# Fanchuana/OPUS-PLLM

Measured on AMD Instinct MI355X. Metric: proteins_per_sec, higher is better.
Workload: dtype f16; 1 GPU; OPUS-PLLM-llama3_8b shape: batch 64/GPU, 512-residue proteins, 89-id prompt (+8 protein tokens = 96 positions), 32 new tokens, greedy (BASELINE configs[3] per-GPU shard: batch 512 over 8 GPUs); batch_per_gpu=64, residues=512, parallelism=replicas x1 (batch-sharded), all-gather of ids

## Files before the change

opus-pllm_amd/csrc/api.cpp:

```cpp
#include "../../include/opus_pllm.h"
#include "common.h"

#include <cmath>
#include <cstdarg>
#include <cstdio>
#include <cstdlib>
#include <cstring>
#include <algorithm>
#include <atomic>
#include <map>
#include <string>
#include <vector>

using namespace opus;

static thread_local char g_err[512] = "";
static int fail(int code, const char *fmt, ...) {
    va_list ap;
    va_start(ap, fmt);
    vsnprintf(g_err, sizeof(g_err), fmt, ap);
    va_end(ap);
    return code;
}
#define HIPC(expr)                                                                                   \
// ... 2409 lines not shown
}

extern "C" int opus_debug_attn_decode(opus_ctx *c, const void *d_qkv, const void *d_k_hist, const void *d_v_hist,
                                      const int32_t *d_kstart, int32_t B, int32_t T0, int32_t step, void *d_out, void *d_k_new,
                                      void *d_v_new, void *stream) {
    if (!c || !d_qkv || !d_kstart || !d_out) return fail(OPUS_EBADARG, "debug_attn_decode: null pointer");
    const opus_config &g = c->cfg;
    const int L = T0 + step, nkv = g.dec_kv_heads, hd = g.dec_head_dim;
    if (B < 1 || B > g.max_batch || T0 < 1 || T0 > g.max_prompt || step < 0 || step >= g.max_new_tokens)
        return fail(OPUS_ESHAPE, "debug_attn_decode: B=%d T0=%d step=%d exceed the context (%d, %d, %d)", B, T0, step, g.max_batch,
                    g.max_prompt, g.max_new_tokens);
    if (L > 0 && (!d_k_hist || !d_v_hist)) return fail(OPUS_EBADARG, "debug_attn_decode: history is null");
    HIPC(hipSetDevice(c->device));
    hipStream_t s = (hipStream_t)stream;
    const size_t pitch = (size_t)c->cache_sh * sizeof(half_t), roww = (size_t)L * hd * sizeof(half_t);
    HIPC(hipMemcpy2DAsync(c->kc, pitch, d_k_hist, roww, roww, (size_t)B * nkv, hipMemcpyDeviceToDevice, s));
    HIPC(hipMemcpy2DAsync(c->vc, pitch, d_v_hist, roww, roww, (size_t)B * nkv, hipMemcpyDeviceToDevice, s));
    HIPC(hipMemcpyAsync(c->d_kstart, d_kstart, (size_t)B * sizeof(int32_t), hipMemcpyDeviceToDevice, s));
    OPC(reset_step(c, s, T0, step));
    HIPC(launch_embed_tokens(c->d_next, nullptr, B, 0, 1, c->d_xl, nullptr, nullptr, 0, c->cs_dec, c->d_kstart, c->d_step, -1, hd / 2,
                             c->cs_row, nullptr, 0, s));
    AttnDecodeParams a;
    a.qkv = (const half_t *)d_qkv; a.slabs = nullptr; a.ks = 0; a.slab_stride = 0; a.row_ssq = nullptr; a.row_nblk = 0; a.eps = 0.f; a.K = 0;
    a.bias = nullptr;
    a.cs_row = c->cs_row; a.kstart = c->d_kstart; a.step = c->d_step; a.T0 = -1; a.nh = g.dec_heads; a.nkv = nkv;
    a.kc = c->kc; a.vc = c->vc; a.cache_sb = c->cache_sb; a.cache_sh = c->cache_sh;
    a.ctx_cap = g.max_prompt + g.max_new_tokens; a.scale = 1.0f / sqrtf((float)hd); a.out = (half_t *)d_out; a.out_tiled = 0;
    c->phase = PH_DECODE;
    KL(KC_ATTN_DECODE, 4.0 * B * nkv * hd * (L + 1), launch_attn_decode(a, B, hd, s));
    const size_t one = (size_t)hd * sizeof(half_t);
    if (d_k_new) HIPC(hipMemcpy2DAsync(d_k_new, one, c->kc + (size_t)L * hd, pitch, one, (size_t)B * nkv, hipMemcpyDeviceToDevice, s));
    if (d_v_new) HIPC(hipMemcpy2DAsync(d_v_new, one, c->vc + (size_t)L * hd, pitch, one, (size_t)B * nkv, hipMemcpyDeviceToDevice, s));
    c->prefilled = false;
    new_epoch(c);
    return OPUS_OK;
}

extern "C" int opus_debug_knob(opus_ctx *c, const char *name, int32_t value) {
    if (!name) return fail(OPUS_EBADARG, "debug_knob: null name");
    if (c) drop_graphs(c);
    if (!strcmp(name, "no_stream")) g_knobs.no_stream = value;
    else if (!strcmp(name, "debug_a_tiled")) g_knobs.debug_a_tiled = value;
    else if (!strcmp(name, "no_ln_fusion")) g_knobs.no_ln_fusion = value;
    else if (!strcmp(name, "enc_full_last_layer")) g_knobs.enc_full_last_layer = value;
    else if (!strcmp(name, "poison_handoff")) {
        if (!c) return fail(OPUS_EBADARG, "poison_handoff needs a context");
        std::vector<int32_t> h(HANDOFF_ERR, 0);
        if (value) for (int i = 0; i < HANDOFF_ERR; ++i) h[i] = i < 512 ? value : ((i & 1) ? 0 : 1);
        HIPC(hipSetDevice(c->device));
        HIPC(hipDeviceSynchronize());
        HIPC(hipMemcpy(c->d_cnt, h.data(), h.size() * sizeof(int32_t), hipMemcpyHostToDevice));
    }
    else if (!strcmp(name, "pp_gm")) { if (value < 1 || value > 64) return fail(OPUS_EBADARG, "pp_gm out of range"); g_knobs.pp_gm = value; }
    else if (!strncmp(name, "misc", 4) && name[4] >= '0' && name[4] <= '7' && !name[5]) g_knobs.misc[name[4] - '0'] = value;
    else return fail(OPUS_EBADARG, "debug_knob: unknown knob '%s'", name);
    return OPUS_OK;
}

extern "C" int64_t opus_stat(opus_ctx *c, const char *name) {
    if (!c || !name) return -1;
    if (!strcmp(name, "graph_instantiations")) return c->graph_instantiations;
    if (!strcmp(name, "graph_replays")) return c->graph_replays;
    if (!strcmp(name, "graphs_cached")) return (int64_t)c->graphs.size();
    if (!strcmp(name, "decode_steps")) return c->decode_steps;
    return -1;
}

extern "C" int opus_timing_enable(opus_ctx *c, int32_t on) {
    if (!c) return fail(OPUS_EBADARG, "ctx is null");
    c->timing = on != 0;
    return OPUS_OK;
}
extern "C" int opus_timing_reset(opus_ctx *c) {
    if (!c) return fail(OPUS_EBADARG, "ctx is null");
    HIPC(hipDeviceSynchronize());
    timing_clear(c);
    return OPUS_OK;
}
static const char *kclass_names[KC_COUNT] = {"gemm_skinny", "gemm_mid", "gemm_wide", "gemm_ring", "gemm_pp", "gemm_tile", "splitk_reduce",
                                            "attn_prefill", "attn_decode", "norm", "other", "gemm_stream", "contact", "constraint", "logitproc",
                                            "xent"};
static const char *phase_names[PH_COUNT] = {"encode", "project", "splice", "prefill", "decode", "other", "score"};

extern "C" int opus_timing_get(opus_ctx *c, const char *kernel_class, const char *phase, double *ms, int64_t *launches,
                               double *bytes, double *flops) {
    if (!c || !kernel_class || !phase || !ms || !launches || !bytes || !flops) return fail(OPUS_EBADARG, "null argument");
    int k = -1, ph = -1;
    const bool any_k = !strcmp(kernel_class, "*"), any_p = !strcmp(phase, "*");
    for (int i = 0; i < KC_COUNT; ++i) if (!strcmp(kclass_names[i], kernel_class)) k = i;
    for (int i = 0; i < PH_COUNT; ++i) if (!strcmp(phase_names[i], phase)) ph = i;
    if (k < 0 && !any_k) return fail(OPUS_EBADARG, "unknown kernel class '%s'", kernel_class);
    if (ph < 0 && !any_p) return fail(OPUS_EBADARG, "unknown phase '%s'", phase);
    HIPC(hipDeviceSynchronize());
    double t = 0, b = 0, f = 0;
    int64_t n = 0;
    for (auto &r : c->recs) {
        if ((!any_k && r.klass != k) || (!any_p && r.phase != ph)) continue;
        float e = 0;
        HIPC(hipEventElapsedTime(&e, r.e0, r.e1));
        t += e;
        b += r.bytes;
        f += r.flops;
        ++n;
    }
    *ms = t;
    *launches = n;
// ... 15 lines not shown
```

opus-pllm_amd/csrc/common.h:

```cpp
#pragma once
#include <hip/hip_runtime.h>
#include <hip/hip_ext.h>
#include <stdint.h>

namespace opus {

#ifdef OPUS_BF16
typedef __bf16 half_t;
typedef __bf16 h8 __attribute__((ext_vector_type(8)));
typedef __bf16 h4 __attribute__((ext_vector_type(4)));
typedef __bf16 h2 __attribute__((ext_vector_type(2)));
#else
typedef _Float16 half_t;
typedef _Float16 h8 __attribute__((ext_vector_type(8)));
typedef _Float16 h4 __attribute__((ext_vector_type(4)));
typedef _Float16 h2 __attribute__((ext_vector_type(2)));
#endif
typedef float f4 __attribute__((ext_vector_type(4)));
__device__ __forceinline__ f4 mfma16(h8 a, h8 b, f4 c) {
#ifdef OPUS_BF16
    return __builtin_amdgcn_mfma_f32_16x16x32_bf16(a, b, c, 0, 0, 0);
#else
    return __builtin_amdgcn_mfma_f32_16x16x32_f16(a, b, c, 0, 0, 0);
#endif
// ... 39 lines not shown
hipError_t ensure_dyn_lds(const void *fn, size_t bytes);

__device__ __forceinline__ void rotate_pair(float a, float b, float c, float sn, float &lo, float &hi) {
    lo = __builtin_fmaf(a, c, -__fmul_rn(b, sn));
    hi = __builtin_fmaf(b, c, __fmul_rn(a, sn));
    asm volatile("" : "+v"(lo), "+v"(hi));
}

__host__ __device__ __forceinline__ int64_t tiled_off(int row, int k, int K) {
    return ((int64_t)(row >> 4) * (K >> 6) + (k >> 6)) * 1024 + ((k & 63) >> 5) * 512 + ((((k & 31) >> 3) << 4) + (row & 15)) * 8 + (k & 7);
}

constexpr int HANDOFF_WORDS = 1024, HANDOFF_ERR = 1023;
constexpr int HANDOFF_SPIN_LIMIT = 1 << 19;

struct GemmParams {
    const half_t *A;
    const float *Af;
    float norm_eps;
    int64_t lda;
    const half_t *W;
    int M, N, K;
    const float *bias;
    const float *residual;
    int64_t ldr;
    void *C;
    int64_t ldc;
    int out_f32;
    int epi;
    float *ws;
    int64_t ws_bytes;
    half_t *xh_out;
    float *ssq_out;
    int *fused_done;
    const float *row_ssq;
    int row_nblk;
    int64_t ssq_cap = 0;
    int *nblk_out = nullptr;
    int slab_only = 0;
    int *ks_out = nullptr;
    int force_wide = 0;
    const float *rope_cs = nullptr;
    const int32_t *rope_pos = nullptr;
    int rope_T = 0, rope_cols = 0, rope_qcols = 0;
    float rope_qscale = 1.0f;
    int *rope_done = nullptr;
    int a_tiled = 0, xh_tiled = 0, c_tiled = 0;
    int *combine_cnt = nullptr;
    float *ln_part = nullptr;
    int *ln_done = nullptr;
    const float *ln_stat = nullptr;
    const float *ln_colsum = nullptr;
    int pp_gm = 8;
    int stagger = 0;
    int no_rot = 0;
    long long *trace = nullptr;
    int *pp_plan = nullptr;
};
constexpr int PP_PLAN_WORDS = 5;
enum PpTail { PP_TAIL_NONE = 0, PP_TAIL_PAIR = 1, PP_TAIL_REDUCE = 2 };

struct AttnParams {
    const half_t *Q, *K, *V;
    int64_t q_sb, q_st, k_sb, k_st, v_sb, v_st;
    half_t *O;
    int64_t o_sb, o_st;
    const int32_t *kstart;
    const int32_t *kend;
    int B, T, heads, group, head_dim, causal;
    float scale;
    const int32_t *cu = nullptr;
    int q_trim = 0;
};

hipError_t launch_gemm(const GemmParams &p, hipStream_t s, int *klass);
hipError_t launch_splitk_reduce(const GemmParams &p, int ks, hipStream_t s);
bool gemm_stream_ok(const GemmParams &p);
bool gemm_stream_would(int M, int N, int K, int slab_only, int a_tiled, int row_scale, int64_t ws_bytes);
hipError_t launch_gemm_stream(const GemmParams &p, hipStream_t s);
struct Knobs {
    int no_stream = 0;
    int no_ln_fusion = 0;
    int debug_a_tiled = 0;
    int pp_gm = 8;
    int enc_full_last_layer = 0;
    int misc[8] = {0, 0, 0, 0, 0, 0, 0, 0};
};
extern Knobs g_knobs;
template <int NWAVES, int ROWS>
__device__ __forceinline__ void block_row_rstd(const float *__restrict__ ssq, int M, int nblk, float inv_k, float eps, float *out,
                                               int wave, int lane) {
    constexpr int RW = (ROWS + NWAVES - 1) / NWAVES;
    float part[RW];
#pragma unroll
    for (int r = 0; r < RW; ++r) part[r] = 0.f;
    for (int j0 = 0; j0 < nblk; j0 += 256) {
        float t[RW][4];
#pragma unroll
        for (int r = 0; r < RW; ++r) {
            int row = wave + NWAVES * r;
            row = row < M ? row : M - 1;
#pragma unroll
            for (int u = 0; u < 4; ++u) {
                const int j = j0 + 64 * u + lane;
                t[r][u] = ssq[(int64_t)row * nblk + (j < nblk ? j : nblk - 1)];
                t[r][u] = j < nblk ? t[r][u] : 0.f;
            }
        }
#pragma unroll
        for (int r = 0; r < RW; ++r) part[r] += (t[r][0] + t[r][1]) + (t[r][2] + t[r][3]);
    }
#pragma unroll
    for (int r = 0; r < RW; ++r) {
        float q = part[r];
#pragma unroll
        for (int o = 32; o > 0; o >>= 1) q += __shfl_xor(q, o, 64);
        const int row = wave + NWAVES * r;
        if (lane == 0 && row < ROWS) out[row] = rsqrtf(q * inv_k + eps);
    }
}
bool gemm_goes_wide(int M, int N);
bool gemm_goes_pp(int M, int N);
hipError_t launch_attn_prefill(const AttnParams &p, hipStream_t s);
struct AttnPrefixParams {
    const half_t *kc, *vc;
    int64_t cache_sb, cache_sh;
    const int32_t *kstart;
    int Tp;
    const half_t *qkv;
    int n;
    const int32_t *list, *off, *blocks;
    half_t *out;
    int nh, nkv, hd;
    float scale;
    const int32_t *par = nullptr;
};
int attn_prefix_blocks(const int32_t *off, int P, int G, int n, int32_t *blocks);
// ... 170 lines not shown
```

opus-pllm_amd/csrc/gemm.hip:

```cpp
#include "common.h"
#include <cstdlib>
#include <map>
#include <type_traits>
#include <mutex>
#include <utility>

namespace opus {

thread_local LaunchEvents *tl_launch_ev = nullptr;
static Knobs knobs_from_env() {
    Knobs k;
    for (int i = 0; i < 8; ++i) {
        char name[32];
        snprintf(name, sizeof(name), "OPUS_KNOB_MISC%d", i);
        if (const char *v = getenv(name)) k.misc[i] = atoi(v);
    }
    return k;
}
Knobs g_knobs = knobs_from_env();

hipError_t ensure_dyn_lds(const void *fn, size_t bytes) {
    static std::mutex mu;
    static std::map<std::pair<int, const void *>, size_t> done;
    int dev = 0;
    hipError_t e = hipGetDevice(&dev);
    if (e != hipSuccess) return e;
    std::lock_guard<std::mutex> lock(mu);
    size_t &have = done[std::make_pair(dev, fn)];
    if (bytes <= have) return hipSuccess;
    e = hipFuncSetAttribute(fn, hipFuncAttributeMaxDynamicSharedMemorySize, (int)bytes);
    if (e == hipSuccess) have = bytes;
    return e;
}

__device__ __forceinline__ float gelu_erf(float x) {
    const float z = fabsf(x) * 0.70710678118654752f;
    const float t = __builtin_amdgcn_rcpf(1.0f + 0.3275911f * z);
    const float poly = t * (0.254829592f + t * (-0.284496736f + t * (1.421413741f + t * (-1.453152027f + t * 1.061405429f))));
    const float erf_abs = 1.0f - poly * __expf(-z * z);
    return 0.5f * x * (1.0f + copysignf(erf_abs, x));
}
__device__ __forceinline__ float silu(float x) { return x * __builtin_amdgcn_rcpf(1.0f + __expf(-x)); }

template <int MT, int EPI, bool NORM, bool ALDS>
__global__ __launch_bounds__(1024) void gemm_skinny_kernel(GemmParams p) {
    extern __shared__ __attribute__((aligned(16))) float red[];
    OPUS_ARGS_ONE_BATCH(p);
    constexpr int PB = EPI == EPI_SILU_GU16 ? 2 : 1;
    const int tid = threadIdx.x;
    const int lane = tid & 63;
    const int wave = __builtin_amdgcn_readfirstlane(tid >> 6);
    const int nwaves = blockDim.x >> 6;
    const int wpp = nwaves / PB;
    const int pl = PB == 1 ? 0 : wave / wpp, kpart = wave - pl * wpp;
    const int chunks = p.K >> 6;
    const int npanels = (p.N + 15) >> 4;
    int panel = blockIdx.x * PB + pl;
    panel = panel < npanels ? panel : npanels - 1;
    const int c0 = kpart_begin(chunks, kpart, wpp);
    const int c1 = kpart_begin(chunks, kpart + 1, wpp);
    const int g = lane >> 4, li = lane & 15;
    float *rss = red + nwaves * MT * 256;
    float *wss = rss + nwaves * MT * 16;
    half_t *xs = reinterpret_cast<half_t *>(wss + 256);
// ... 713 lines not shown
        if (ks + 1 < KS) read_frags(ks + 1, na, nb);
        __builtin_amdgcn_sched_barrier(0);
        mfmas(ca, cb, 1, TM);
        __builtin_amdgcn_s_setprio(0);
    };
    h8 a0[TM], b0[TN], a1[TM], b1[TN];
#pragma unroll
    for (int s = 0; s < NS; ++s)
        if (s < KS) stage_load(s);
    wait_glds(issued_upto(NS - 1));
    __builtin_amdgcn_s_barrier();
    read_frags(0, a0, b0);
    for (int ks = 0; ks < KS; ks += 2) {
        step(ks, a0, b0, a1, b1);
        if (ks + 1 < KS) step(ks + 1, a1, b1, a0, b0);
    }

    if (ksplit > 1) {
        float *slab = p.ws + (int64_t)ky * p.M * p.N;
#pragma unroll
        for (int i = 0; i < TM; ++i) {
            const int m = m0 + wm * (16 * TM) + i * 16 + li;
            if (m >= p.M) continue;
#pragma unroll
            for (int j = 0; j < TN; ++j) {
                const int nb = n0 + wn * (16 * TN) + j * 16 + 4 * g;
                if ((p.N & 3) == 0 && nb + 3 < p.N) {
                    *reinterpret_cast<float4 *>(slab + (int64_t)m * p.N + nb) = make_float4(acc[i][j][0], acc[i][j][1], acc[i][j][2], acc[i][j][3]);
                } else {
#pragma unroll
                    for (int r = 0; r < 4; ++r)
                        if (nb + r < p.N) slab[(int64_t)m * p.N + nb + r] = acc[i][j][r];
                }
            }
        }
        return;
    }
#pragma unroll
    for (int i = 0; i < TM; ++i) {
        const int m = m0 + wm * (16 * TM) + i * 16 + li;
        if (m >= p.M) continue;
        if (EPI == EPI_SILU_GU16) {
#pragma unroll
            for (int jj = 0; jj < TN / 2; ++jj)
                store4<EPI>(p, m, n0 + wn * (16 * TN) + jj * 32 + 4 * g, acc[i][2 * jj], acc[i][2 * jj + 1]);
        } else {
#pragma unroll
            for (int j = 0; j < TN; ++j) store4<EPI>(p, m, n0 + wn * (16 * TN) + j * 16 + 4 * g, acc[i][j], acc[i][j]);
        }
    }
}

constexpr int PP_DIST = 6;

__host__ __device__ __forceinline__ void pp_tile_coords(int id, int tiles_m, int tiles_n, int &tm, int &tn, int GM = 8) {
    const int per_group = GM * tiles_n;
    const int grp = id / per_group, rem_id = id - grp * per_group;
    const int rows_here = (tiles_m - grp * GM) < GM ? (tiles_m - grp * GM) : GM;
    tm = grp * GM + rem_id % rows_here;
    tn = rem_id / rows_here;
}
template <int EPI, bool LNA>
__device__ __forceinline__ void pp_finish(const GemmParams &p, f4 (&acc)[8][4], char *smem, const int wave, const int m0, const int n0,
                                          const int bid, const int full_tiles, const int tail_split, const int kpart, const bool partial);
template <int EPI, bool LNA>
__device__ __forceinline__ void pp_epilogue(const GemmParams &p, f4 (&acc)[8][4], char *smem, const int wave, const int m0, const int n0,
                                            const char *pair_slab);
template <int EPI, bool LNA = false>
__global__ __launch_bounds__(512) void gemm_pp_kernel(GemmParams p, int tiles_m, int tiles_n, int full_tiles, int tail_split) {
    extern __shared__ __attribute__((aligned(16))) char smem[];
    constexpr int HT = 16384;
    const int tid = threadIdx.x, lane = tid & 63;
    const int wave = __builtin_amdgcn_readfirstlane(tid >> 6);
    const int wr = wave >> 2, wc = wave & 3;
    const int g = lane >> 4, li = lane & 15;
    if (p.stagger > 0 && blockIdx.x < 256 && ((blockIdx.x >> 3) & 1))
        for (int i = 0; i < p.stagger; ++i) __builtin_amdgcn_s_sleep(127);
    if (p.trace && tid == 0) p.trace[blockIdx.x * 4] = wall_clock64();
    int bid = blockIdx.x, kpart = 0;
    const bool partial = bid >= full_tiles;
    if (!partial) {
        const int nwg = full_tiles, q = nwg >> 3, rr = nwg & 7, xcd = bid & 7;
        bid = (xcd < rr ? xcd * (q + 1) : rr * (q + 1) + (xcd - rr) * q) + (bid >> 3);
    } else {
        const int j = bid - full_tiles;
        bid = full_tiles + j / tail_split;
        kpart = j % tail_split;
    }
    int tm, tn;
    pp_tile_coords(bid, tiles_m, tiles_n, tm, tn, p.pp_gm);
    const int m0 = tm * 256, n0 = tn * 256;
    const int KT_all = p.K >> 6;
    const int kt0 = partial ? (int)((int64_t)KT_all * kpart / tail_split) : 0;
    const int kt1 = partial ? (int)((int64_t)KT_all * (kpart + 1) / tail_split) : KT_all;
    const int KT = kt1 - kt0, NH = 4 * KT;
    const int npanels = (p.N + 15) >> 4;

    typedef const __attribute__((address_space(1))) void *gptr_t;
    typedef __attribute__((address_space(3))) void *lptr_t;
    unsigned offA[2][2], offB[2][2];
#pragma unroll
    for (int j = 0; j < 2; ++j) {
        const int q = 2 * wave + j;
        const int lr = 8 * q + (lane >> 3);
        const int chunk = (lane & 7) ^ ((lr >> 1) & 7);
#pragma unroll
        for (int rh = 0; rh < 2; ++rh) {
            int row = m0 + (lr >> 6) * 128 + rh * 64 + (lr & 63);
            row = row < p.M ? row : p.M - 1;
            offA[j][rh] = (unsigned)(((int64_t)row * p.lda + chunk * 8) * 2);
        }
        const int pi = q >> 1, s = q & 1;
#pragma unroll
        for (int ch = 0; ch < 2; ++ch) {
            int pn = (n0 >> 4) + (pi >> 1) * 4 + ch * 2 + (pi & 1);
            pn = pn < npanels ? pn : npanels - 1;
            offB[j][ch] = (unsigned)((((int64_t)pn * KT_all) * 1024 + s * 512 + lane * 8) * 2);
        }
    }
    const char *baseA = reinterpret_cast<const char *>(p.A) + (int64_t)kt0 * 128;
    const char *baseB = reinterpret_cast<const char *>(p.W) + (int64_t)kt0 * 2048;
    auto issue_half = [&](int hq) {
        const int kt = hq >> 2, i = hq & 3;
        char *dst = smem + (hq & 7) * HT + (2 * wave) * 1024;
        const char *sa = baseA + (int64_t)kt * 128, *sb = baseB + (int64_t)kt * 2048;
#pragma unroll
        for (int j = 0; j < 2; ++j) {
            const char *src = (i == 0 || i == 3) ? sa + offA[j][i == 3] : sb + offB[j][i == 2];
            __builtin_amdgcn_global_load_lds((gptr_t)src, (lptr_t)(dst + j * 1024), 16, 0, 0);
        }
    };

// ... 10 lines not shown
#pragma unroll
        for (int s = 0; s < 2; ++s) aoff[rt][s] = lr * 128 + (((4 * s + g) ^ ((lr >> 1) & 7)) << 4);
    }
    const int boff = (wc * 2) * 2048 + lane * 16;
    auto read_a = [&](int kt, int rh, h8 (&af)[4][2]) {
        const char *base = smem + (4 * (kt & 1) + (rh ? 3 : 0)) * HT;
#pragma unroll
        for (int rt = 0; rt < 4; ++rt)
#pragma unroll
            for (int s = 0; s < 2; ++s) af[rt][s] = *reinterpret_cast<const h8 *>(base + aoff[rt][s]);
    };
    auto read_b = [&](int kt, int ch, h8 (&bf)[2][2]) {
        const char *base = smem + (4 * (kt & 1) + 1 + ch) * HT + boff;
#pragma unroll
        for (int ct = 0; ct < 2; ++ct)
#pragma unroll
            for (int s = 0; s < 2; ++s) bf[ct][s] = *reinterpret_cast<const h8 *>(base + ct * 2048 + s * 1024);
    };
    auto mfma_quadrant = [&](int rh, int ch, const h8 (&af)[4][2], const h8 (&bf)[2][2]) {
        asm volatile("s_waitcnt lgkmcnt(0)" ::: "memory");
        __builtin_amdgcn_s_setprio(1);
#pragma unroll
        for (int rt = 0; rt < 4; ++rt)
#pragma unroll
            for (int ct = 0; ct < 2; ++ct)
#pragma unroll
                for (int s = 0; s < 2; ++s) {
#pragma unroll
                    for (int rhh = 0; rhh < 2; ++rhh)
#pragma unroll
                        for (int chh = 0; chh < 2; ++chh)
                            if (rhh == rh && chh == ch)
                                acc[4 * rhh + rt][2 * chh + ct] =
                                    mfma16(bf[ct][s], af[rt][s], acc[4 * rhh + rt][2 * chh + ct]);
                }
        __builtin_amdgcn_s_setprio(0);
    };
    constexpr int D = PP_DIST;
    auto feed = [&](int phi) {
        if (phi + D < NH) {
            issue_half(phi + D);
            vmcnt_wait<2 * (D - 2)>();
        } else {
            const int left = NH - 1 - (phi + 2);
            if (left >= 3) vmcnt_wait<6>();
            else if (left == 2) vmcnt_wait<4>();
            else if (left == 1) vmcnt_wait<2>();
            else vmcnt_wait<0>();
        }
    };

#pragma unroll
    for (int h = 0; h < D; ++h)
        if (h < NH) issue_half(h);
    if (NH >= D) vmcnt_wait<2 * (D - 4)>();
    else vmcnt_wait<0>();
    __builtin_amdgcn_s_barrier();
    if (p.trace && tid == 0) p.trace[blockIdx.x * 4 + 1] = wall_clock64();
    if (wr == 1) __builtin_amdgcn_s_barrier();
    read_a(0, 0, a0);

    for (int kt = 0; kt < KT; ++kt) {
        const int phi = 4 * kt;
        read_b(kt, 0, b0);
        feed(phi);
        __builtin_amdgcn_s_barrier();
        mfma_quadrant(0, 0, a0, b0);
        __builtin_amdgcn_s_barrier();
        read_b(kt, 1, b1);
        feed(phi + 1);
        __builtin_amdgcn_s_barrier();
        mfma_quadrant(0, 1, a0, b1);
        __builtin_amdgcn_s_barrier();
        read_a(kt, 1, a1);
        feed(phi + 2);
        __builtin_amdgcn_s_barrier();
        mfma_quadrant(1, 1, a1, b1);
        __builtin_amdgcn_s_barrier();
        if (kt + 1 < KT) read_a(kt + 1, 0, a0);
        feed(phi + 3);
        __builtin_amdgcn_s_barrier();
        mfma_quadrant(1, 0, a1, b0);
        __builtin_amdgcn_s_barrier();
    }
    if (wr == 0) __builtin_amdgcn_s_barrier();
    if (p.trace && tid == 0) p.trace[blockIdx.x * 4 + 2] = wall_clock64();
    pp_finish<EPI, LNA>(p, acc, smem, wave, m0, n0, bid, full_tiles, tail_split, kpart, partial);
}

template <int EPI, bool LNA>
__device__ __forceinline__ void pp_finish(const GemmParams &p, f4 (&acc)[8][4], char *smem, const int wave, const int m0, const int n0,
                                          const int bid, const int full_tiles, const int tail_split, const int kpart, const bool partial) {
    int lane;
    asm volatile("v_mbcnt_lo_u32_b32 %0, -1, 0\n\tv_mbcnt_hi_u32_b32 %0, -1, %0" : "=v"(lane));
    const int tid = wave * 64 + lane;
    const int wr = wave >> 2, wc = wave & 3;
    const int g = lane >> 4, li = lane & 15;

    const char *pair_slab = nullptr;
    if (partial && tail_split == 2 && p.combine_cnt) {
        typedef unsigned int u4p __attribute__((ext_vector_type(4)));
        const int tt = bid - full_tiles;
        int *cnt = p.combine_cnt + 512 + 2 * tt;
        int *word = reinterpret_cast<int *>(smem);
        if (tid == 0) *word = __hip_atomic_fetch_add(cnt, 1, __ATOMIC_RELAXED, __HIP_MEMORY_SCOPE_AGENT);
        __syncthreads();
        const int order = *word;
        __syncthreads();
        if (order > 1 && tid == 0)
            __hip_atomic_store(p.combine_cnt + HANDOFF_ERR, 1, __ATOMIC_RELAXED, __HIP_MEMORY_SCOPE_AGENT);
        const __amdgpu_buffer_rsrc_t srs = __builtin_amdgcn_make_buffer_rsrc((void *)(p.ws + ((int64_t)tt << 16)), 0, 1 << 18, 0x00020000);
        if (order == 0) {
#pragma unroll
            for (int i = 0; i < 8; ++i)
#pragma unroll
                for (int j = 0; j < 4; ++j)
                    __builtin_amdgcn_raw_buffer_store_b128(__builtin_bit_cast(u4p, acc[i][j]), srs, ((i * 4 + j) * 512 + tid) * 16, 0, 16);
            asm volatile("s_waitcnt vmcnt(0)" ::: "memory");
            __syncthreads();
            if (tid == 0) __hip_atomic_store(cnt + 1, 1, __ATOMIC_RELAXED, __HIP_MEMORY_SCOPE_AGENT);
            return;
        }
        if (tid == 0) {
            int spins = 0;
            while (__hip_atomic_load(cnt + 1, __ATOMIC_RELAXED, __HIP_MEMORY_SCOPE_AGENT) == 0) {
                __builtin_amdgcn_s_sleep(4);
                if (++spins > HANDOFF_SPIN_LIMIT) {
                    __hip_atomic_store(p.combine_cnt + HANDOFF_ERR, 1, __ATOMIC_RELAXED, __HIP_MEMORY_SCOPE_AGENT);
                    break;
                }
            }
            __hip_atomic_store(cnt, 0, __ATOMIC_RELAXED, __HIP_MEMORY_SCOPE_AGENT);
            __hip_atomic_store(cnt + 1, 0, __ATOMIC_RELAXED, __HIP_MEMORY_SCOPE_AGENT);
        }
        __syncthreads();
        pair_slab = reinterpret_cast<const char *>(p.ws + ((int64_t)tt << 16));
    } else if (partial) {
        float *slab = p.ws + (((int64_t)(bid - full_tiles) * tail_split + kpart) << 16);
#pragma unroll
        for (int i = 0; i < 8; ++i) {
            const int r = wr * 128 + i * 16 + li;
#pragma unroll
            for (int j = 0; j < 4; ++j)
                *reinterpret_cast<float4 *>(slab + r * 256 + wc * 64 + j * 16 + 4 * g) = make_float4(acc[i][j][0], acc[i][j][1], acc[i][j][2], acc[i][j][3]);
        }
        return;
    }
    pp_epilogue<EPI, LNA>(p, acc, smem, wave, m0, n0, pair_slab);
}

template <int EPI, bool LNA>
__device__ __forceinline__ void pp_epilogue(const GemmParams &p, f4 (&acc)[8][4], char *smem, const int wave, const int m0, const int n0,
                                            const char *pair_slab) {
    int lane;
    asm volatile("v_mbcnt_lo_u32_b32 %0, -1, 0\n\tv_mbcnt_hi_u32_b32 %0, -1, %0" : "=v"(lane));
    const int tid = wave * 64 + lane;
    const int wr = wave >> 2, wc = wave & 3;
    const int g = lane >> 4, li = lane & 15;
    constexpr int NO = EPI == EPI_SILU_GU16 ? 32 : 64;
    const int nlim = EPI == EPI_SILU_GU16 ? p.N / 2 : p.N;
    const int nw0 = EPI == EPI_SILU_GU16 ? (n0 >> 1) + wc * 32 : n0 + wc * 64;
    const bool rows16 = ((p.ldc & 7) == 0) && ((p.ldr & 3) == 0) && nw0 + NO <= nlim;
    const __amdgpu_buffer_rsrc_t psrs = __builtin_amdgcn_make_buffer_rsrc((void *)pair_slab, 0, pair_slab ? 1 << 18 : 0, 0x00020000);
    auto pair_load = [&](int i, int j) {
        return __builtin_bit_cast(f4, __builtin_amdgcn_raw_buffer_load_b128(psrs, ((i * 4 + j) * 512 + tid) * 16, 0, 16));
    };
    if (!rows16) {
#pragma unroll
        for (int i = 0; i < 8; ++i) {
            f4 av[4];
#pragma unroll
            for (int j = 0; j < 4; ++j) av[j] = acc[i][j];
            if (pair_slab) {
#pragma unroll
                for (int j = 0; j < 4; ++j) av[j] += pair_load(i, j);
            }
            const int m = m0 + wr * 128 + i * 16 + li;
            if (m >= p.M) continue;
            if (EPI == EPI_SILU_GU16) {
#pragma unroll
                for (int jj = 0; jj < 2; ++jj) store4<EPI>(p, m, n0 + wc * 64 + jj * 32 + 4 * g, av[2 * jj], av[2 * jj + 1]);
            } else {
#pragma unroll
                for (int j = 0; j < 4; ++j) store4<EPI>(p, m, n0 + wc * 64 + j * 16 + 4 * g, av[j], av[j]);
            }
        }
        return;
    }
    float *patch = reinterpret_cast<float *>(smem + wave * 16384);
    constexpr bool XSW = NO == 64;
    constexpr int PS = XSW ? NO : NO + 4;
    auto pidx = [&](int r, int c) { return XSW ? r * PS + ((((c >> 2) ^ (r & 15)) << 2) | (c & 3)) : r * PS + c; };
    float bz[16];
#pragma unroll
    for (int q = 0; q < 16; ++q) bz[q] = 0.f;
    if (p.bias && !LNA && EPI == EPI_SILU_GU16) {
        if (EPI == EPI_SILU_GU16) {
#pragma unroll
            for (int jj = 0; jj < 2; ++jj)
#pragma unroll
                for (int r = 0; r < 4; ++r) {
                    const int nb = n0 + wc * 64 + jj * 32 + 4 * g + r;
                    bz[jj * 8 + r] = p.bias[nb];
                    bz[jj * 8 + 4 + r] = p.bias[nb + 16];
                }
        } else {
#pragma unroll
            for (int j = 0; j < 4; ++j)
#pragma unroll
                for (int r = 0; r < 4; ++r) bz[j * 4 + r] = p.bias[n0 + wc * 64 + j * 16 + 4 * g + r];
        }
    }
    float *cb = patch + 2048;
    float2 lst[2][2];
    auto load_stat = [&](int i, float2 &st) {
        int m = m0 + wr * 128 + i * 16 + li;
        m = m < p.M ? m : p.M - 1;
        st = reinterpret_cast<const float2 *>(p.ln_stat)[m];
    };
    if constexpr (EPI != EPI_SILU_GU16) {
        const int nc = n0 + wc * 64 + lane;
        cb[lane] = (p.bias && nc < p.N) ? p.bias[nc] : 0.f;
        if constexpr (LNA) cb[64 + lane] = p.ln_colsum ? p.ln_colsum[nc] : 0.f;
    }
    if constexpr (LNA) {
        load_stat(0, lst[0][0]);
        load_stat(1, lst[0][1]);
    }
    constexpr int LPR32 = NO / 4, RPP32 = 64 / LPR32, LPR16 = NO / 8, RPP16 = 64 / LPR16;
    constexpr int NR = (16 / RPP32) > 2 * (16 / RPP16) ? (16 / RPP32) : 2 * (16 / RPP16);
    auto load_res = [&](int i, float4 (&rr)[NR]) {
        const int mrow0 = m0 + wr * 128 + i * 16;
        if (p.out_f32) {
#pragma unroll
            for (int ps = 0; ps < 16 / RPP32; ++ps) {
                const int r = ps * RPP32 + lane / LPR32, c = (lane % LPR32) * 4;
                const int m = mrow0 + r < p.M ? mrow0 + r : p.M - 1;
                rr[ps] = *reinterpret_cast<const float4 *>(p.residual + (int64_t)m * p.ldr + nw0 + c);
            }
        } else {
#pragma unroll
            for (int ps = 0; ps < 16 / RPP16; ++ps) {
// ... 181 lines not shown
                            ohi[e] = (half_t)rh;
                        }
                        const int off = ((tr0 + r) * (int)p.ldc + nw0 + c) * 2;
                        __builtin_amdgcn_raw_buffer_store_b128(__builtin_bit_cast(u4v, olo), crs, off, 0, 0);
                        __builtin_amdgcn_raw_buffer_store_b128(__builtin_bit_cast(u4v, ohi), crs, off + 64, 0, 0);
                    }
                } else {
#pragma unroll
                    for (int ps = 0; ps < 16 / RPP16; ++ps) {
                        const int r = ps * RPP16 + lane / LPR16, c = (lane % LPR16) * 8;
                        f4 lo = *reinterpret_cast<const f4 *>(pu + pidx(r, c)), hi = *reinterpret_cast<const f4 *>(pu + pidx(r, c + 4));
                        if constexpr (MODE == M_GENERIC) {
                            const float4 r0 = rcur[2 * ps], r1 = rcur[2 * ps + 1];
                            lo[0] += r0.x; lo[1] += r0.y; lo[2] += r0.z; lo[3] += r0.w;
                            hi[0] += r1.x; hi[1] += r1.y; hi[2] += r1.z; hi[3] += r1.w;
                        }
                        const h8 o = h8{(half_t)lo[0], (half_t)lo[1], (half_t)lo[2], (half_t)lo[3], (half_t)hi[0], (half_t)hi[1], (half_t)hi[2], (half_t)hi[3]};
                        __builtin_amdgcn_raw_buffer_store_b128(__builtin_bit_cast(u4v, o), crs, ((tr0 + r) * (int)p.ldc + nw0 + c) * 2, 0, 0);
                    }
                }
            }
            asm volatile("s_waitcnt lgkmcnt(0)" ::: "memory");
            if constexpr (PAIR) {
                if (ib + 1 < 8 / RB) prefetch(ib + 1);
            }
        }
    };
    typedef std::false_type NP;
    typedef std::true_type WP;
    if constexpr (LNA) {
        if (rope_on) run(std::integral_constant<int, ROPE_OK ? M_ROPE : M_F16>{}, NP{});
        else if (pair_slab) run(std::integral_constant<int, M_F16>{}, WP{});
        else run(std::integral_constant<int, M_F16>{}, NP{});
    } else if constexpr (EPI != EPI_NONE) {
        if (!p.out_f32 && !p.residual) {
            if (pair_slab) run(std::integral_constant<int, M_F16>{}, WP{});
            else run(std::integral_constant<int, M_F16>{}, NP{});
        } else run(std::integral_constant<int, M_GENERIC>{}, NP{});
    } else {
        if (rope_on) run(std::integral_constant<int, M_ROPE>{}, NP{});
        else if (!p.out_f32 && !p.residual) {
            if (pair_slab) run(std::integral_constant<int, M_F16>{}, WP{});
            else run(std::integral_constant<int, M_F16>{}, NP{});
        } else if (p.out_f32 && p.residual && p.ln_part) {
            if (pair_slab) run(std::integral_constant<int, M_F32RES_LN>{}, WP{});
            else run(std::integral_constant<int, M_F32RES_LN>{}, NP{});
        } else if (p.out_f32 && p.residual) {
            if (pair_slab) run(std::integral_constant<int, M_F32RES>{}, WP{});
            else run(std::integral_constant<int, M_F32RES>{}, NP{});
        } else run(std::integral_constant<int, M_GENERIC>{}, NP{});
    }
    if (p.trace && tid == 0) {
        asm volatile("s_waitcnt vmcnt(0)" ::: "memory");
        p.trace[blockIdx.x * 4 + 3] = wall_clock64();
    }
}

template <int EPI>
__global__ __launch_bounds__(256) void pp_tail_reduce_kernel(GemmParams p, int tiles_m, int tiles_n, int full_tiles, int tail_split) {
    int tm, tn;
    pp_tile_coords(full_tiles + blockIdx.x, tiles_m, tiles_n, tm, tn, p.pp_gm);
    const int lane = threadIdx.x & 63, wave = threadIdx.x >> 6;
    const int col = 4 * lane, n = tn * 256 + col;
    const float *base = p.ws + ((int64_t)blockIdx.x * tail_split << 16) + col;
    f4 bias4 = f4{0.f, 0.f, 0.f, 0.f}, bias_up = f4{0.f, 0.f, 0.f, 0.f};
    const bool gate_lane = (col & 31) < 16;
    if (p.bias) {
#pragma unroll
        for (int c = 0; c < 4; ++c) {
            if (n + c < p.N) bias4[c] = p.bias[n + c];
            if (EPI == EPI_SILU_GU16 && gate_lane && n + 16 + c < p.N) bias_up[c] = p.bias[n + 16 + c];
        }
    }
    constexpr int RW = 8;
    f4 csum = f4{0.f, 0.f, 0.f, 0.f};
    if (p.ln_stat && p.ln_colsum) {
#pragma unroll
        for (int c = 0; c < 4; ++c)
            if (n + c < p.N) csum[c] = p.ln_colsum[n + c];
    }
    f4 v[RW];
#pragma unroll
    for (int i = 0; i < RW; ++i) v[i] = f4{0.f, 0.f, 0.f, 0.f};
    const int r0 = blockIdx.y * 32 + wave * RW;
    for (int k0 = 0; k0 < tail_split; k0 += 4) {
        float4 t[4][RW];
#pragma unroll
        for (int u = 0; u < 4; ++u) {
            const int kk = k0 + u < tail_split ? k0 + u : tail_split - 1;
#pragma unroll
            for (int i = 0; i < RW; ++i) t[u][i] = *reinterpret_cast<const float4 *>(base + ((int64_t)kk << 16) + (r0 + i) * 256);
        }
#pragma unroll
        for (int u = 0; u < 4; ++u) {
            if (k0 + u >= tail_split) continue;
#pragma unroll
            for (int i = 0; i < RW; ++i) { v[i][0] += t[u][i].x; v[i][1] += t[u][i].y; v[i][2] += t[u][i].z; v[i][3] += t[u][i].w; }
        }
    }
    const int no_v = EPI == EPI_SILU_GU16 ? ((n >> 5) << 4) + (n & 15) : n;
    const bool vec_ok = no_v + 3 < (EPI == EPI_SILU_GU16 ? p.N / 2 : p.N) && ((p.ldc | p.ldr) & 3) == 0;
    float4 rres[RW];
#pragma unroll
    for (int i = 0; i < RW; ++i) {
        const int m = tm * 256 + r0 + i;
        rres[i] = make_float4(0.f, 0.f, 0.f, 0.f);
        if (p.residual && vec_ok && m < p.M) rres[i] = *reinterpret_cast<const float4 *>(p.residual + (int64_t)m * p.ldr + no_v);
// ... 16 lines not shown
        } else {
            float2 st = make_float2(0.f, 1.f);
            if (p.ln_stat) st = reinterpret_cast<const float2 *>(p.ln_stat)[m < p.M ? m : p.M - 1];
#pragma unroll
            for (int c = 0; c < 4; ++c) {
                x[c] = p.ln_stat ? __builtin_fmaf(st.y, x[c] - st.x * csum[c], bias4[c]) : x[c] + bias4[c];
                if (EPI == EPI_GELU) x[c] = gelu_erf(x[c]);
            }
            live = live && n < p.N;
        }
        if (!live) continue;
        const int nlim = EPI == EPI_SILU_GU16 ? p.N / 2 : p.N;
        if (vec_ok) {
            if (p.residual) {
                const float4 rr = rres[i];
                x[0] += rr.x; x[1] += rr.y; x[2] += rr.z; x[3] += rr.w;
            }
            if (p.out_f32) *reinterpret_cast<float4 *>(reinterpret_cast<float *>(p.C) + (int64_t)m * p.ldc + no) = make_float4(x[0], x[1], x[2], x[3]);
            else *reinterpret_cast<h4 *>(reinterpret_cast<half_t *>(p.C) + (int64_t)m * p.ldc + no) = h4{(half_t)x[0], (half_t)x[1], (half_t)x[2], (half_t)x[3]};
            if (EPI == EPI_NONE && p.ln_part) {
                *reinterpret_cast<h4 *>(p.xh_out + (int64_t)m * p.N + no) = h4{(half_t)x[0], (half_t)x[1], (half_t)x[2], (half_t)x[3]};
                float s1 = (x[0] + x[1]) + (x[2] + x[3]);
                float s2 = (x[0] * x[0] + x[1] * x[1]) + (x[2] * x[2] + x[3] * x[3]);
#pragma unroll
                for (int o = 1; o < 16; o <<= 1) { s1 += __shfl_xor(s1, o, 64); s2 += __shfl_xor(s2, o, 64); }
                if ((lane & 15) == 0) reinterpret_cast<float2 *>(p.ln_part)[(int64_t)m * (p.N >> 6) + (no >> 6)] = make_float2(s1, s2);
            }
        } else {
#pragma unroll
            for (int c = 0; c < 4; ++c) {
                if (no + c >= nlim) continue;
                float y = x[c];
                if (p.residual) y += p.residual[(int64_t)m * p.ldr + no + c];
                if (p.out_f32) reinterpret_cast<float *>(p.C)[(int64_t)m * p.ldc + no + c] = y;
                else reinterpret_cast<half_t *>(p.C)[(int64_t)m * p.ldc + no + c] = (half_t)y;
            }
        }
    }
}

template <int EPI>
static hipError_t launch_pp(const GemmParams &p_in, hipStream_t s) {
    if (p_in.row_ssq) return hipErrorInvalidValue;
    if ((int64_t)p_in.M * p_in.lda * 2 >= (1ll << 32) || (int64_t)p_in.N * p_in.K * 2 >= (1ll << 32)) return hipErrorInvalidValue;
    GemmParams p = p_in;
    const bool lna = p.ln_stat != nullptr;
    if (lna && (p.out_f32 || p.residual || (p.N & 255) || (p.ldc & 7) || (EPI == EPI_SILU_GU16 && (p.bias || p.ln_colsum)))) return hipErrorInvalidValue;
    const bool lnp = p.ln_part && p.xh_out && p.ln_done && EPI == EPI_NONE && p.out_f32 && (p.N & 255) == 0 && (p.ldc & 7) == 0 &&
                     (p.ldr & 3) == 0 && p.residual;
    if (lnp) *p.ln_done = 1;
    else p.ln_part = nullptr;
    p.stagger = g_knobs.misc[5];
    p.pp_gm = g_knobs.pp_gm;
    void (*kern)(GemmParams, int, int, int, int) = gemm_pp_kernel<EPI, false>;
    if (lna) kern = gemm_pp_kernel<EPI, true>;
    const int bm = cdiv(p.M, 256), bn = cdiv(p.N, 256);
    hipError_t ea = ensure_dyn_lds(reinterpret_cast<const void *>(kern), 8 * 16384);
    if (ea != hipSuccess) return ea;
    const int T = bm * bn, KT = p.K >> 6;
    int full = T, split = 1;
    static const bool no_tail = getenv("OPUS_NO_PP_TAIL") != nullptr;
    static const bool no_rope_fuse = getenv("OPUS_NO_ROPE_FUSION") != nullptr;
    const bool rope = p.rope_cs && p.rope_done && !no_rope_fuse && EPI == EPI_NONE && !p.out_f32 && !p.residual && (p.ldc & 7) == 0 &&
                      (p.N & 255) == 0 && (p.rope_cols & 63) == 0 && (p.rope_qcols & 63) == 0 && p.rope_T > 0;
    if (rope) *p.rope_done = 1;
    else p.rope_cs = nullptr;
    const int R = T % 256;
    if (!no_tail && !rope && p.ws && T > 256 && R > 0 && R <= 128) {
        int sp = 256 / R;
        sp = sp > 8 ? 8 : sp;
        if (sp > KT / 4) sp = KT / 4;
        while (sp > 1 && ((int64_t)R * sp << 18) > p.ws_bytes) --sp;
        const double t_tile = 1.5 * KT + 12.0, gain = t_tile * (1.0 - 1.0 / sp), cost = (sp == 2 && p.combine_cnt && !g_knobs.misc[6]) ? 22.0 : 30.0;
        if (sp > 1 && gain > cost) { full = T - R; split = sp; }
    }
    const int tail = T - full;
    static const bool trace = getenv("OPUS_PP_TRACE") != nullptr;
    if (trace) {
        static long long *tb = nullptr;
        const int nwg = full + tail * split;
        if (!tb) (void)hipMalloc((void **)&tb, (size_t)(1 << 16) * 4 * sizeof(long long));
        if (tb && nwg <= (1 << 16)) {
            GemmParams q = p;
            q.trace = tb;
            hipLaunchKernelGGL(kern, dim3(nwg), dim3(512), 8 * 16384, s, q, bm, bn, full, split);
            (void)hipStreamSynchronize(s);
            std::vector<long long> h((size_t)nwg * 4);
            (void)hipMemcpy(h.data(), tb, h.size() * sizeof(long long), hipMemcpyDeviceToHost);
            long long t0 = h[0], t1 = h[3];
            double pro = 0, mainl = 0, epi = 0;
            for (int i = 0; i < nwg; ++i) {
                t0 = std::min(t0, h[4 * i]); t1 = std::max(t1, h[4 * i + 3]);
                if (i < full) { pro += h[4 * i + 1] - h[4 * i]; mainl += h[4 * i + 2] - h[4 * i + 1]; epi += h[4 * i + 3] - h[4 * i + 2]; }
            }
            fprintf(stderr, "[pp trace] M=%d N=%d K=%d epi=%d wg=%d (full %d): kernel %.1f us; per full tile: prologue %.2f us, main %.2f us, epilogue %.2f us\n",
                    p.M, p.N, p.K, EPI, nwg, full, (t1 - t0) * 0.01, pro / full * 0.01, mainl / full * 0.01, epi / full * 0.01);
            for (int r0 = 0; r0 < nwg; r0 += 256) {
                double st = 0, en = 0; int n = 0;
                for (int i = r0; i < nwg && i < r0 + 256; ++i, ++n) { st += h[4 * i] - t0; en += h[4 * i + 3] - t0; }
                fprintf(stderr, "   wg %5d..: mean start %.1f us, mean end %.1f us\n", r0, st / n * 0.01, en / n * 0.01);
            }
        }
    }
    const bool pair_mode = (!p.out_f32 && !p.residual) || (EPI == EPI_NONE && p.out_f32 && p.residual);
    const bool pair = split == 2 && p.combine_cnt && !g_knobs.misc[6] && pair_mode && (p.ldc & 7) == 0 && (p.ldr & 3) == 0 && (p.N & 255) == 0;
    if (!pair) p.combine_cnt = nullptr;
    if (p.pp_plan) {
        p.pp_plan[0] = full; p.pp_plan[1] = tail; p.pp_plan[2] = split;
        p.pp_plan[3] = split == 1 ? PP_TAIL_NONE : pair ? PP_TAIL_PAIR : PP_TAIL_REDUCE;
        p.pp_plan[4] = rope ? 1 : 0;
    }
    OPUS_LAUNCH(KC_PP, kern, dim3(full + tail * split), dim3(512), 8 * 16384, s, p, bm, bn, full, split);
    hipError_t e = hipGetLastError();
    if (e != hipSuccess || split == 1 || pair) return e;
    if (tl_launch_ev) tl_launch_ev->aux_bytes = ((double)tail * split * 65536 * 4) + (double)tail * 65536 * (p.out_f32 ? 4 : 2);
    OPUS_LAUNCH(KC_REDUCE, (pp_tail_reduce_kernel<EPI>), dim3(tail, 8), dim3(256), 0, s, p, bm, bn, full, split);
    return hipGetLastError();
}

template <int EPI>
__global__ __launch_bounds__(256) void splitk_reduce_kernel(GemmParams p, int ksplit) {
    const int nout = EPI == EPI_SILU_GU16 ? p.N / 2 : p.N;
    const int64_t i = (int64_t)blockIdx.x * 256 + threadIdx.x;
    if (i >= (int64_t)p.M * nout) return;
    const int m = (int)(i / nout), no = (int)(i % nout);
    const int64_t slab = (int64_t)p.M * p.N;
    float rstd = 1.0f;
    if (p.Af) {
        float q = 0.f;
        for (int k = 0; k < ksplit; ++k) q += p.ws[ksplit * slab + (int64_t)k * p.M + m];
        rstd = rsqrtf(q / (float)p.K + p.norm_eps);
    } else if (p.row_ssq) {
        const float *src = p.row_ssq + (int64_t)m * p.row_nblk;
        float q0 = 0.f, q1 = 0.f, q2 = 0.f, q3 = 0.f;
        int j = 0;
        for (; j + 4 <= p.row_nblk; j += 4) { q0 += src[j]; q1 += src[j + 1]; q2 += src[j + 2]; q3 += src[j + 3]; }
        for (; j < p.row_nblk; ++j) q0 += src[j];
        rstd = rsqrtf(((q0 + q1) + (q2 + q3)) / (float)p.K + p.norm_eps);
    }
    float v;
    if (EPI == EPI_SILU_GU16) {
        const int n = (no >> 4) * 32 + (no & 15);
        float gate = 0.f, up = 0.f;
        for (int k0 = 0; k0 < ksplit; k0 += 8) {
            float tg[8], tu[8];
#pragma unroll
            for (int u = 0; u < 8; ++u) {
                const int kk = k0 + u < ksplit ? k0 + u : ksplit - 1;
                tg[u] = p.ws[kk * slab + (int64_t)m * p.N + n];
                tu[u] = p.ws[kk * slab + (int64_t)m * p.N + n + 16];
            }
#pragma unroll
            for (int u = 0; u < 8; ++u)
                if (k0 + u < ksplit) { gate += tg[u]; up += tu[u]; }
        }
        gate *= rstd;
        up *= rstd;
        if (p.bias) { gate += p.bias[n]; up += p.bias[n + 16]; }
        v = silu(gate) * up;
    } else {
        v = 0.f;
        for (int k0 = 0; k0 < ksplit; k0 += 8) {
            float t[8];
#pragma unroll
            for (int u = 0; u < 8; ++u) {
// ... 538 lines not shown
```

Measured before the change: 260.8 proteins/s.

## Make gemm_pp persistent with cross-tile prefetch of next tile's first K-stages

Converts the ping-pong GEMM kernel into a resident kernel that launches at most 256 workgroups, each looping over full tiles in strides of 256. Before running its epilogue, a workgroup now issues async global-to-LDS loads for the first five K stages of its next tile. This overlaps the next tile's prologue with the current epilogue and avoids workgroup launch and teardown costs. In exchange, LDS grows to 10x16KB and the epilogue patch buffer moves to a separate region, which can lower occupancy and adds risk in the index arithmetic and barrier handling.

Result: no change. 258.6 proteins/s (-0.9%).

```diff
diff --git a/opus-pllm_amd/csrc/api.cpp b/opus-pllm_amd/csrc/api.cpp
--- a/opus-pllm_amd/csrc/api.cpp
+++ b/opus-pllm_amd/csrc/api.cpp
@@ -2485,6 +2485,8 @@
         HIPC(hipMemcpy(c->d_cnt, h.data(), h.size() * sizeof(int32_t), hipMemcpyHostToDevice));
     }
     else if (!strcmp(name, "pp_gm")) { if (value < 1 || value > 64) return fail(OPUS_EBADARG, "pp_gm out of range"); g_knobs.pp_gm = value; }
+    else if (!strcmp(name, "pp_resident")) g_knobs.pp_resident = value != 0;
+    else if (!strcmp(name, "pp_prefetch")) g_knobs.pp_prefetch = value != 0;
     else if (!strncmp(name, "misc", 4) && name[4] >= '0' && name[4] <= '7' && !name[5]) g_knobs.misc[name[4] - '0'] = value;
     else return fail(OPUS_EBADARG, "debug_knob: unknown knob '%s'", name);
     return OPUS_OK;
diff --git a/opus-pllm_amd/csrc/common.h b/opus-pllm_amd/csrc/common.h
--- a/opus-pllm_amd/csrc/common.h
+++ b/opus-pllm_amd/csrc/common.h
@@ -115,6 +115,8 @@
     const float *ln_stat = nullptr;
     const float *ln_colsum = nullptr;
     int pp_gm = 8;
+    int pp_resident = 1;
+    int pp_prefetch = 1;
     int stagger = 0;
     int no_rot = 0;
     long long *trace = nullptr;
@@ -146,6 +148,8 @@
     int no_ln_fusion = 0;
     int debug_a_tiled = 0;
     int pp_gm = 8;
+    int pp_resident = 1;
+    int pp_prefetch = 1;
     int enc_full_last_layer = 0;
     int misc[8] = {0, 0, 0, 0, 0, 0, 0, 0};
 };
diff --git a/opus-pllm_amd/csrc/gemm.hip b/opus-pllm_amd/csrc/gemm.hip
--- a/opus-pllm_amd/csrc/gemm.hip
+++ b/opus-pllm_amd/csrc/gemm.hip
@@ -10,6 +10,8 @@
 thread_local LaunchEvents *tl_launch_ev = nullptr;
 static Knobs knobs_from_env() {
     Knobs k;
+    if (const char *v = getenv("OPUS_PP_RESIDENT")) k.pp_resident = atoi(v) != 0;
+    if (const char *v = getenv("OPUS_PP_PREFETCH")) k.pp_prefetch = atoi(v) != 0;
     for (int i = 0; i < 8; ++i) {
         char name[32];
         snprintf(name, sizeof(name), "OPUS_KNOB_MISC%d", i);
@@ -829,6 +831,8 @@
 }
 
 constexpr int PP_DIST = 6;
+constexpr int PP_AHEAD = 5, PP_PATCH = 8704, PP_LDS = 10 * 16384;
+static_assert(PP_AHEAD < PP_DIST && PP_AHEAD * 16384 + 8 * PP_PATCH <= PP_LDS, "gemm_pp LDS plan");
 
 __host__ __device__ __forceinline__ void pp_tile_coords(int id, int tiles_m, int tiles_n, int &tm, int &tn, int GM = 8) {
     const int per_group = GM * tiles_n;
@@ -839,22 +843,22 @@
 }
 template <int EPI, bool LNA>
 __device__ __forceinline__ void pp_finish(const GemmParams &p, f4 (&acc)[8][4], char *smem, const int wave, const int m0, const int n0,
-                                          const int bid, const int full_tiles, const int tail_split, const int kpart, const bool partial);
+                                          const int bid, const int full_tiles, const int tail_split, const int kpart, const bool partial,
+                                          const int vid);
 template <int EPI, bool LNA>
 __device__ __forceinline__ void pp_epilogue(const GemmParams &p, f4 (&acc)[8][4], char *smem, const int wave, const int m0, const int n0,
-                                            const char *pair_slab);
-template <int EPI, bool LNA = false>
-__global__ __launch_bounds__(512) void gemm_pp_kernel(GemmParams p, int tiles_m, int tiles_n, int full_tiles, int tail_split) {
-    extern __shared__ __attribute__((aligned(16))) char smem[];
+                                            const char *pair_slab, const int vid);
+template <int EPI, bool LNA>
+__device__ __forceinline__ void pp_tile(const GemmParams &p, char *smem, const int wave, const int vid, const int tiles_m, const int tiles_n,
+                                        const int full_tiles, const int tail_split, const bool pre, const bool nxt) {
     constexpr int HT = 16384;
-    const int tid = threadIdx.x, lane = tid & 63;
-    const int wave = __builtin_amdgcn_readfirstlane(tid >> 6);
+    int lane;
+    asm volatile("v_mbcnt_lo_u32_b32 %0, -1, 0\n\tv_mbcnt_hi_u32_b32 %0, -1, %0" : "=v"(lane));
+    const int tid = wave * 64 + lane;
     const int wr = wave >> 2, wc = wave & 3;
     const int g = lane >> 4, li = lane & 15;
-    if (p.stagger > 0 && blockIdx.x < 256 && ((blockIdx.x >> 3) & 1))
-        for (int i = 0; i < p.stagger; ++i) __builtin_amdgcn_s_sleep(127);
-    if (p.trace && tid == 0) p.trace[blockIdx.x * 4] = wall_clock64();
-    int bid = blockIdx.x, kpart = 0;
+    if (p.trace && tid == 0) p.trace[vid * 4] = wall_clock64();
+    int bid = vid, kpart = 0;
     const bool partial = bid >= full_tiles;
     if (!partial) {
         const int nwg = full_tiles, q = nwg >> 3, rr = nwg & 7, xcd = bid & 7;
@@ -971,11 +975,11 @@
 
 #pragma unroll
     for (int h = 0; h < D; ++h)
-        if (h < NH) issue_half(h);
+        if (h < NH && !(pre && h < PP_AHEAD)) issue_half(h);
     if (NH >= D) vmcnt_wait<2 * (D - 4)>();
     else vmcnt_wait<0>();
     __builtin_amdgcn_s_barrier();
-    if (p.trace && tid == 0) p.trace[blockIdx.x * 4 + 1] = wall_clock64();
+    if (p.trace && tid == 0) p.trace[vid * 4 + 1] = wall_clock64();
     if (wr == 1) __builtin_amdgcn_s_barrier();
     read_a(0, 0, a0);
 
@@ -1003,13 +1007,81 @@
         __builtin_amdgcn_s_barrier();
     }
     if (wr == 0) __builtin_amdgcn_s_barrier();
-    if (p.trace && tid == 0) p.trace[blockIdx.x * 4 + 2] = wall_clock64();
-    pp_finish<EPI, LNA>(p, acc, smem, wave, m0, n0, bid, full_tiles, tail_split, kpart, partial);
+    if (p.trace && tid == 0) p.trace[vid * 4 + 2] = wall_clock64();
+    if (nxt) {
+        int ln;
+        asm volatile("v_mbcnt_lo_u32_b32 %0, -1, 0\n\tv_mbcnt_hi_u32_b32 %0, -1, %0" : "=v"(ln));
+        int nb = vid + 256;
+        {
+            const int nwg = full_tiles, q = nwg >> 3, rr = nwg & 7, xcd = nb & 7;
+            nb = (xcd < rr ? xcd * (q + 1) : rr * (q + 1) + (xcd - rr) * q) + (nb >> 3);
+        }
+        int tm2, tn2;
+        pp_tile_coords(nb, tiles_m, tiles_n, tm2, tn2, p.pp_gm);
+#pragma unroll
+        for (int j = 0; j < 2; ++j) {
+            const int q = 2 * wave + j;
+            const int lr = 8 * q + (ln >> 3);
+            const int chunk = (ln & 7) ^ ((lr >> 1) & 7);
+            const int pi = q >> 1, sh = q & 1;
+#pragma unroll
+            for (int h = 0; h < PP_AHEAD; ++h) {
+                if (h >= NH) continue;
+                const int i = h & 3;
+                unsigned off;
+                if (i == 0 || i == 3) {
+                    int row = tm2 * 256 + (lr >> 6) * 128 + (i == 3) * 64 + (lr & 63);
+                    row = row < p.M ? row : p.M - 1;
+                    off = (unsigned)(((int64_t)row * p.lda + chunk * 8) * 2);
+                } else {
+                    int pn = tn2 * 16 + (pi >> 1) * 4 + (i == 2) * 2 + (pi & 1);
+                    pn = pn < npanels ? pn : npanels - 1;
+                    off = (unsigned)((((int64_t)pn * KT_all) * 1024 + sh * 512 + ln * 8) * 2);
+                }
+                const char *src = (i == 0 || i == 3) ? reinterpret_cast<const char *>(p.A) + (int64_t)(h >> 2) * 128 + off
+                                                     : reinterpret_cast<const char *>(p.W) + (int64_t)(h >> 2) * 2048 + off;
+                __builtin_amdgcn_global_load_lds((gptr_t)src, (lptr_t)(smem + h * HT + q * 1024), 16, 0, 0);
+            }
+        }
+    }
+    pp_finish<EPI, LNA>(p, acc, smem, wave, m0, n0, bid, full_tiles, tail_split, kpart, partial, vid);
+}
+
+template <int EPI, bool LNA = false>
+__global__ __launch_bounds__(512) void gemm_pp_kernel(GemmParams p, int tiles_m, int tiles_n, int full_tiles, int tail_split) {
+    extern __shared__ __attribute__((aligned(16))) char smem[];
+    const int wave = __builtin_amdgcn_readfirstlane(threadIdx.x >> 6);
+    if (p.stagger > 0 && blockIdx.x < 256 && ((blockIdx.x >> 3) & 1))
+        for (int i = 0; i < p.stagger; ++i) __builtin_amdgcn_s_sleep(127);
+    int vid = blockIdx.x;
+    {
+        const int nres = full_tiles < 256 ? full_tiles : 256;
+        if (p.pp_resident && vid >= nres) vid += full_tiles - nres;
+    }
+    struct PpArgs { GemmParams p; int tiles_m, tiles_n, full_tiles, tail_split; };
+    typedef const __attribute__((address_space(4))) PpArgs *kargs_t;
+    for (;;) {
+        kargs_t ka = (kargs_t)__builtin_amdgcn_kernarg_segment_ptr();
+        asm volatile("" : "+s"(ka));
+        const PpArgs &a = *(const PpArgs *)ka;
+        int w = wave;
+        asm volatile("" : "+s"(w));
+        const bool pf = a.p.pp_resident && a.p.pp_prefetch && vid < a.full_tiles;
+        pp_tile<EPI, LNA>(a.p, smem, w, vid, a.tiles_m, a.tiles_n, a.full_tiles, a.tail_split, pf && vid >= 256, pf && vid + 256 < a.full_tiles);
+        kargs_t kb = (kargs_t)__builtin_amdgcn_kernarg_segment_ptr();
+        asm volatile("" : "+s"(kb));
+        const PpArgs &b = *(const PpArgs *)kb;
+        vid += 256;
+        if (!b.p.pp_resident || vid >= b.full_tiles) break;
+        asm volatile("s_waitcnt lgkmcnt(0)" ::: "memory");
+        __builtin_amdgcn_s_barrier();
+    }
 }
 
 template <int EPI, bool LNA>
 __device__ __forceinline__ void pp_finish(const GemmParams &p, f4 (&acc)[8][4], char *smem, const int wave, const int m0, const int n0,
-                                          const int bid, const int full_tiles, const int tail_split, const int kpart, const bool partial) {
+                                          const int bid, const int full_tiles, const int tail_split, const int kpart, const bool partial,
+                                          const int vid) {
     int lane;
     asm volatile("v_mbcnt_lo_u32_b32 %0, -1, 0\n\tv_mbcnt_hi_u32_b32 %0, -1, %0" : "=v"(lane));
     const int tid = wave * 64 + lane;
@@ -1065,12 +1137,12 @@
         }
         return;
     }
-    pp_epilogue<EPI, LNA>(p, acc, smem, wave, m0, n0, pair_slab);
+    pp_epilogue<EPI, LNA>(p, acc, smem, wave, m0, n0, pair_slab, vid);
 }
 
 template <int EPI, bool LNA>
 __device__ __forceinline__ void pp_epilogue(const GemmParams &p, f4 (&acc)[8][4], char *smem, const int wave, const int m0, const int n0,
-                                            const char *pair_slab) {
+                                            const char *pair_slab, const int vid) {
     int lane;
     asm volatile("v_mbcnt_lo_u32_b32 %0, -1, 0\n\tv_mbcnt_hi_u32_b32 %0, -1, %0" : "=v"(lane));
     const int tid = wave * 64 + lane;
@@ -1106,7 +1178,7 @@
         }
         return;
     }
-    float *patch = reinterpret_cast<float *>(smem + wave * 16384);
+    float *patch = reinterpret_cast<float *>(smem + PP_AHEAD * 16384 + wave * PP_PATCH);
     constexpr bool XSW = NO == 64;
     constexpr int PS = XSW ? NO : NO + 4;
     auto pidx = [&](int r, int c) { return XSW ? r * PS + ((((c >> 2) ^ (r & 15)) << 2) | (c & 3)) : r * PS + c; };
@@ -1394,7 +1466,7 @@
     }
     if (p.trace && tid == 0) {
         asm volatile("s_waitcnt vmcnt(0)" ::: "memory");
-        p.trace[blockIdx.x * 4 + 3] = wall_clock64();
+        p.trace[vid * 4 + 3] = wall_clock64();
     }
 }
 
@@ -1517,10 +1589,12 @@
     else p.ln_part = nullptr;
     p.stagger = g_knobs.misc[5];
     p.pp_gm = g_knobs.pp_gm;
+    p.pp_resident = g_knobs.pp_resident;
+    p.pp_prefetch = g_knobs.pp_prefetch;
     void (*kern)(GemmParams, int, int, int, int) = gemm_pp_kernel<EPI, false>;
     if (lna) kern = gemm_pp_kernel<EPI, true>;
     const int bm = cdiv(p.M, 256), bn = cdiv(p.N, 256);
-    hipError_t ea = ensure_dyn_lds(reinterpret_cast<const void *>(kern), 8 * 16384);
+    hipError_t ea = ensure_dyn_lds(reinterpret_cast<const void *>(kern), PP_LDS);
     if (ea != hipSuccess) return ea;
     const int T = bm * bn, KT = p.K >> 6;
     int full = T, split = 1;
@@ -1540,6 +1614,7 @@
         if (sp > 1 && gain > cost) { full = T - R; split = sp; }
     }
     const int tail = T - full;
+    const int grid = (p.pp_resident ? std::min(full, 256) : full) + tail * split;
     static const bool trace = getenv("OPUS_PP_TRACE") != nullptr;
     if (trace) {
         static long long *tb = nullptr;
@@ -1548,7 +1623,7 @@
         if (tb && nwg <= (1 << 16)) {
             GemmParams q = p;
             q.trace = tb;
-            hipLaunchKernelGGL(kern, dim3(nwg), dim3(512), 8 * 16384, s, q, bm, bn, full, split);
+            hipLaunchKernelGGL(kern, dim3(grid), dim3(512), PP_LDS, s, q, bm, bn, full, split);
             (void)hipStreamSynchronize(s);
             std::vector<long long> h((size_t)nwg * 4);
             (void)hipMemcpy(h.data(), tb, h.size() * sizeof(long long), hipMemcpyDeviceToHost);
@@ -1575,7 +1650,7 @@
         p.pp_plan[3] = split == 1 ? PP_TAIL_NONE : pair ? PP_TAIL_PAIR : PP_TAIL_REDUCE;
         p.pp_plan[4] = rope ? 1 : 0;
     }
-    OPUS_LAUNCH(KC_PP, kern, dim3(full + tail * split), dim3(512), 8 * 16384, s, p, bm, bn, full, split);
+    OPUS_LAUNCH(KC_PP, kern, dim3(grid), dim3(512), PP_LDS, s, p, bm, bn, full, split);
     hipError_t e = hipGetLastError();
     if (e != hipSuccess || split == 1 || pair) return e;
     if (tl_launch_ev) tl_launch_ev->aux_bytes = ((double)tail * split * 65536 * 4) + (double)tail * 65536 * (p.out_f32 ? 4 : 2);
```
